# MIT-SPARK/Khronos

Measured on AMD Instinct MI355X. Metric: active-window frames/sec (+ Mvoxel-updates/sec) at 1280x720 RGB-D+labels, 2 cm voxels, higher is better.
Workload: dtype f32

## Files before the change

### khronos_amd/csrc/khr_kernels_fuse.h

```cpp
#pragma once
#include "khr_device.h"

namespace khr {

__device__ inline void interpPixels(float u, float v, int W, int H, int* px, float* du, float* dv) {
  const int u0 = static_cast<int>(floorf(u)), v0 = static_cast<int>(floorf(v));
  const int u1 = min(u0 + 1, W - 1), v1 = min(v0 + 1, H - 1);
  *du = u - static_cast<float>(u0);
  *dv = v - static_cast<float>(v0);
  px[0] = v0 * W + u0;
  px[1] = v1 * W + u0;
  px[2] = v0 * W + u1;
  px[3] = v1 * W + u1;
}

__device__ inline int interpWeights(float du, float dv, bool use_nearest, float* w4) {
  int best;
  if (use_nearest) {
    const int nearest = (du >= 0.5f ? 2 : 0) + (dv >= 0.5f ? 1 : 0);
#pragma unroll
    for (int k = 0; k < 4; ++k) w4[k] = (k == nearest) ? 1.f : 0.f;
    best = nearest;
  } else {
    w4[0] = (1.f - du) * (1.f - dv);
// ... 369 lines not shown
  __syncthreads();
  char* const sink_b = reinterpret_cast<char*>(a.sink) + (static_cast<size_t>(blockIdx.x) * WPW + static_cast<size_t>(wave)) * 256u;
  const bool trk = a.with_tracking != 0;
  const uint32_t first = (blockIdx.x & 7u) * (gridDim.x >> 3) + (blockIdx.x >> 3);
  auto pull = [&]() -> uint32_t {
    uint32_t j = 0u;
    if (lane == 0) j = atomicAdd(&s_q, 1u);
    j = static_cast<uint32_t>(__builtin_amdgcn_readfirstlane(static_cast<int>(j)));
    return first + gridDim.x * j;
  };
  auto descOf = [&](uint32_t i) -> uint4 {
    typedef const FuseList __attribute__((address_space(4))) * FuseListK;
    const char __attribute__((address_space(4)))* kb = (const char __attribute__((address_space(4)))*)__builtin_amdgcn_kernarg_segment_ptr();
    asm volatile("" : "+s"(kb));
    const FuseListK kl = (FuseListK)(kb + ((sizeof(FuseArgs) + 7u) & ~static_cast<size_t>(7)));
    const uint32_t __attribute__((address_space(4)))* const kc = (const uint32_t __attribute__((address_space(4)))*)kl->counts;
    const uint32_t c0 = kc[0], c1 = c0 + kc[1], c2 = c1 + kc[2];
    const DescK la = (DescK)kl->a, lb = (DescK)kl->b;
    const uint32_t cap = kl->cap;
    u4v d;
    if (i < c0) d = la[i];
    else if (i < c1) d = la[cap - 1u - (i - c0)];
    else if (i < c2) d = lb[i - c1];
    else d = lb[cap - 1u - (i - c2)];
    return make_uint4(d.x, d.y, d.z, d.w);
  };

  auto phase1 = [&](FuseItem<VPS, ZR>& it, const uint4 desc) {
    const uint32_t dx = static_cast<uint32_t>(__builtin_amdgcn_readfirstlane(static_cast<int>(desc.x)));
    it.slot = dx & 0xffffffu;
    it.sbi = static_cast<int>(dx >> 24);
    const int bx = __builtin_amdgcn_readfirstlane(static_cast<int>(desc.y));
    const int by = __builtin_amdgcn_readfirstlane(static_cast<int>(desc.z));
    const int bz = __builtin_amdgcn_readfirstlane(static_cast<int>(desc.w));
    const int patch = it.sbi % PATCHES;
    it.z0 = (it.sbi / PATCHES) * ZR;
    const float ox = static_cast<float>(bx) * a.bs, oy = static_cast<float>(by) * a.bs;
    it.oz = static_cast<float>(bz) * a.bs;
    it.lin_xy = patch * 64 + lane;
    const int ix = it.lin_xy % VPS, iy = it.lin_xy / VPS;
    const float px = ox + (static_cast<float>(ix) + 0.5f) * a.vs;
    const float py = oy + (static_cast<float>(iy) + 0.5f) * a.vs;
    float pxy[3];
#pragma unroll
    for (int c = 0; c < 3; ++c) pxy[c] = a.R[3 * c] * px + a.R[3 * c + 1] * py;
    it.pxy2 = pxy[2];
    const char* const dist_b = reinterpret_cast<const char*>(a.dist + it.slot * NV);
    const char* const wgt_b = reinterpret_cast<const char*>(a.weight + it.slot * NV);
#pragma unroll
    for (int k = 0; k < ZR; ++k) {
      const int iz = it.z0 + k;
      const uint32_t lin = static_cast<uint32_t>(it.lin_xy + iz * SL);
      const float pz = it.oz + (static_cast<float>(iz) + 0.5f) * a.vs;
      float pc[3];
#pragma unroll
      for (int c = 0; c < 3; ++c) pc[c] = (pxy[c] + a.R[3 * c + 2] * pz) + a.t[c];
      bool ok = pc[2] > 0.f;
      const float voxel_range = range_mode == 0 ? pc[2] : sqrtf((pc[0] * pc[0] + pc[1] * pc[1]) + pc[2] * pc[2]);
      ok = ok && !(voxel_range < a.min_range || voxel_range > a.max_range);
      const float yz = rcpRefined(pc[2]);
      const float u = divExact(pc[0] * a.fx, pc[2], yz) + a.cx;
      const float v = divExact(pc[1] * a.fy, pc[2], yz) + a.cy;
      ok = ok && (fminf(fminf(u, v), fminf(Wm1 - u, Hm1 - v)) >= 0.f);
      const float uc = ok ? u : 0.f, vc = ok ? v : 0.f;
      const uint32_t u0 = static_cast<uint32_t>(static_cast<int>(uc)), v0 = static_cast<uint32_t>(static_cast<int>(vc));
      const uint32_t v1 = min(v0 + 1u, static_cast<uint32_t>(a.H - 1));
      const uint32_t o0 = __umul24(v0, W4) + u0 * 4u, o1 = __umul24(v1, W4) + u0 * 4u;
      it.ra[k] = *reinterpret_cast<const f2u*>(range_b + o0);
      it.rb[k] = *reinterpret_cast<const f2u*>(range_b + o1);
      it.d[k] = *reinterpret_cast<const float*>(dist_b + lin * 4u);
      it.w[k] = *reinterpret_cast<const float*>(wgt_b + lin * 4u);
      it.u[k] = uc;
      it.v[k] = vc;
      it.z[k] = ok ? voxel_range : -1.f;
      it.yz[k] = yz;
    }
  };

  auto phase2 = [&](FuseItem<VPS, ZR>& cur) {
    const size_t slot = cur.slot;
    char* const dist_b = reinterpret_cast<char*>(a.dist + slot * NV);
    char* const wgt_b = reinterpret_cast<char*>(a.weight + slot * NV);
    char* const lobs_b = reinterpret_cast<char*>(a.last_obs + slot * NV);
    uint32_t cnt = 0;
    bool touched = false;
    bool wrote_neg = false;
    const size_t w0 = slot * static_cast<size_t>(NV / 64) + static_cast<size_t>(cur.z0 * PATCHES + cur.sbi % PATCHES);
    u4v ow_next = trk ? ((DescK)(a.obs + w0))[0] : u4v{0u, 0u, 0u, 0u};
#pragma unroll
    for (int k = 0; k < ZR; ++k) {
      const u4v ow_k = ow_next;
      if (k + 1 < ZR && trk) ow_next = ((DescK)(a.obs + w0))[(k + 1) * PATCHES];
      bool ok = cur.z[k] >= 0.f;
      const int iz = cur.z0 + k;
      const uint32_t lin = static_cast<uint32_t>(cur.lin_xy + iz * SL);
      const float d_old = cur.d[k], w_old = cur.w[k];
      float d_out = d_old, w_out = w_old;
      if (__builtin_amdgcn_ballot_w64(ok) != 0ull) {
      const float uc = cur.u[k], vc = cur.v[k], voxel_range = cur.z[k], yz = cur.yz[k];
      float depth = voxel_range;
      if (range_mode != 0) {
        const float pz = cur.oz + (static_cast<float>(iz) + 0.5f) * a.vs;
        depth = (cur.pxy2 + a.R[8] * pz) + a.t[2];
      }
      const uint32_t u0 = static_cast<uint32_t>(static_cast<int>(uc)), v0 = static_cast<uint32_t>(static_cast<int>(vc));
      const uint32_t v1 = min(v0 + 1u, static_cast<uint32_t>(a.H - 1));
      const float du = __builtin_amdgcn_fractf(uc), dv = __builtin_amdgcn_fractf(vc);
      const uint32_t o0 = v0 * W4 + u0 * 4u, o1 = v1 * W4 + u0 * 4u;
      const bool last_col = u0 >= static_cast<uint32_t>(a.W - 1);
      const float r0 = cur.ra[k].x, r1 = cur.rb[k].x, r2 = last_col ? cur.ra[k].x : cur.ra[k].y, r3 = last_col ? cur.rb[k].x : cur.rb[k].y;
      bool use_nearest = interp == 0;
      if (interp == 2) {
        const float mn = fminf(fminf(r0, r1), fminf(r2, r3));
        const float mx = fmaxf(fmaxf(r0, r1), fmaxf(r2, r3));
        use_nearest = use_nearest || (mx - mn > a.adaptive_diff);
      }
      const bool hi_u = du >= 0.5f, hi_v = dv >= 0.5f;
      const float r_near = hi_u ? (hi_v ? r3 : r2) : (hi_v ? r1 : r0);
      const float omu = 1.f - du, omv = 1.f - dv;
      const float w0 = omu * omv, w1 = omu * dv, w2 = du * omv, w3 = du * dv;
      const float r_bil = ((w0 * r0 + w1 * r1) + w2 * r2) + w3 * r3;
      const float dist_surface = use_nearest ? r_near : r_bil;
      ok = ok && (dist_surface >= a.min_range) && !(dist_surface > a.max_range);
      const float sdf = dist_surface - voxel_range;
      ok = ok && !(sdf < -a.trunc);
      bool in_band = ok && (fabsf(sdf) < a.trunc);
      if (__builtin_expect(a.use_mask && __builtin_amdgcn_ballot_w64(in_band) != 0ull, 0)) {
        int best;
        if (use_nearest) {
          best = (hi_u ? 2 : 0) + (hi_v ? 1 : 0);
        } else {
          best = 0;
          float bw = w0;
          if (w1 > bw) { bw = w1; best = 1; }
          if (w2 > bw) { bw = w2; best = 2; }
          if (w3 > bw) { bw = w3; best = 3; }
        }
        const uint32_t uo = ((best & 2) && !last_col) ? 4u : 0u;
        const uint32_t bo = ((best & 1) ? o1 : o0) + uo;
        if (in_band && *reinterpret_cast<const int32_t*>(reinterpret_cast<const char*>(a.dyn) + bo) != 0) {
          ok = false;
          in_band = false;
        }
      }
      if (__builtin_amdgcn_ballot_w64(ok) != 0ull) {
      float w;
      if (EXACT) {
        const float qd = divExact(a.vs, depth, yz);
        w = fxfy * (qd * qd);
        if (!const_weight) {
          const float z2 = depth * depth;
          w = divExact(w, z2, rcpRefined(z2));
        }
        if (use_dropoff && sdf < -a.dropoff_eps) w = fmaxf(w * divExact(a.trunc + sdf, den, yden), 0.f);
      } else {
        const float qd = a.vs * yz;
        w = fxfy * (qd * qd);
        if (!const_weight) w = w * (yz * yz);
        if (use_dropoff && sdf < -a.dropoff_eps) w = fmaxf(w * ((a.trunc + sdf) * yden), 0.f);
      }
      ok = ok && (w > 0.f);
      in_band = in_band && ok;
      const float sdf_c = fmaxf(fminf(a.trunc, sdf), -a.trunc);
      const float tot = w_old + w;
      float d_new;
      if (EXACT) {
        d_new = divExact(d_old * w_old + sdf_c * w, tot, rcpRefined(tot));
      } else {
        d_new = __builtin_fmaf(d_old, w_old, sdf_c * w) * __builtin_amdgcn_rcpf(tot);
      }
      const float w_new = fminf(tot, a.max_weight);
      if (ok) {
        d_out = d_new;
        w_out = w_new;
      }
      const unsigned long long m_band = __builtin_amdgcn_ballot_w64(in_band);
      wrote_neg = wrote_neg || (__builtin_amdgcn_ballot_w64(ok && d_new < 0.f) != 0ull);
      if (m_band) {
        n_band += static_cast<uint32_t>(__popcll(m_band));
        if (in_band) {
          const uint32_t pos = cnt + __builtin_amdgcn_mbcnt_hi(static_cast<uint32_t>(m_band >> 32),
                                                              __builtin_amdgcn_mbcnt_lo(static_cast<uint32_t>(m_band), 0u));
          uint32_t* const rec = &s_rec[wave][0][pos];
          rec[0] = lin | (use_nearest ? 0x10000u : 0u);
          rec[kRecCap] = __float_as_uint(w);
          rec[2 * kRecCap] = __float_as_uint(a.blend_pre ? w_old : w_new);
          rec[3 * kRecCap] = __float_as_uint(uc);
          rec[4 * kRecCap] = __float_as_uint(vc);
        }
        cnt += static_cast<uint32_t>(__popcll(m_band));
      }
      } else {
        ok = false;
      }
      }
      const unsigned long long m_ok = __builtin_amdgcn_ballot_w64(ok);
      n_upd += static_cast<uint32_t>(__popcll(m_ok));
      touched = touched || (m_ok != 0ull);
      {
        char* const d_b = m_ok != 0ull ? dist_b : sink_b;
        char* const w_b = m_ok != 0ull ? wgt_b : sink_b;
        const uint32_t vo = (m_ok != 0ull ? lin : static_cast<uint32_t>(lane)) * 4u;
        *reinterpret_cast<float*>(d_b + vo) = d_out;
        *reinterpret_cast<float*>(w_b + vo) = w_out;
      }
      {
        const uint64_t bits0 = static_cast<uint64_t>(ow_k.x) | (static_cast<uint64_t>(ow_k.y) << 32);
        const uint64_t stamp0 = static_cast<uint64_t>(ow_k.z) | (static_cast<uint64_t>(ow_k.w) << 32);
        const bool same = stamp0 == a.stamp;
        const uint64_t mat = (m_ok != 0ull && !same) ? (bits0 & ~m_ok) : 0ull;
        const uint64_t nb = m_ok == 0ull ? bits0 : (same ? (bits0 | m_ok) : m_ok);
        const uint64_t ns = m_ok == 0ull ? stamp0 : a.stamp;
        const bool real = trk && mat != 0ull;
        char* const st_b = real ? lobs_b : sink_b;
        const uint32_t first_lin = lin - static_cast<uint32_t>(lane) + static_cast<uint32_t>(__builtin_ctzll(mat | (1ull << 63)));
        const bool mine = ((mat >> static_cast<uint32_t>(lane)) & 1ull) != 0ull;
        const uint32_t so = real ? (mine ? lin : first_lin) * 8u : 0u;
        *reinterpret_cast<uint64_t*>(st_b + so) = stamp0;
        ulonglong2* const wp = trk ? (a.obs + w0 + k * PATCHES) : reinterpret_cast<ulonglong2*>(sink_b + 16);
        *wp = make_ulonglong2(nb, ns);
      }
    }
    const uint32_t item_band = cnt;
    if (__builtin_expect(cnt > 0u, 0)) {
      __builtin_amdgcn_fence(__ATOMIC_RELEASE, "wavefront");
      __builtin_amdgcn_wave_barrier();
      FuseArgsK ka = (FuseArgsK)__builtin_amdgcn_kernarg_segment_ptr();
      asm volatile("" : "+s"(ka));
      const FuseFrameK kf = (FuseFrameK)ka;
      if (ka->band_mode != 0 && fuseBandRowsOk(ka->KS, ka->sem_mode, ka->do_sem, ka->has_color)) {
        fuseBandRows<VPS>(ka, kf, slot, &s_rec[wave][0][0], cnt, lane);
      } else {
        for (uint32_t r = static_cast<uint32_t>(lane); r < cnt; r += 64u) {
          const uint32_t* const rec = &s_rec[wave][0][r];
          fuseBandRecord<VPS>(ka, kf, slot, rec[0], __uint_as_float(rec[kRecCap]), __uint_as_float(rec[2 * kRecCap]),
                              __uint_as_float(rec[3 * kRecCap]), __uint_as_float(rec[4 * kRecCap]));
        }
      }
      __builtin_amdgcn_fence(__ATOMIC_ACQUIRE, "wavefront");
      __builtin_amdgcn_wave_barrier();
      __builtin_amdgcn_s_waitcnt(0x0f70);
    }
    {
      const uint32_t recw = min(item_band, static_cast<uint32_t>(kItemBandMask)) | (touched ? kItemTouched : 0u) | (wrote_neg ? kItemNeg : 0u);
      a.blk_band[slot * kBandSlots + (cur.sbi & (kBandSlots - 1))] = static_cast<uint16_t>(recw);
    }
  };

  uint32_t item = pull();
  if (item < n_items) {
    FuseItem<VPS, ZR> sa, sb;
    uint4 d_cur = descOf(item);
    phase1(sa, d_cur);
    uint32_t item_next = pull();
    uint4 d_next = item_next < n_items ? descOf(item_next) : d_cur;
    while (true) {
      {
        phase1(sb, d_next);
        const uint32_t item_nn = item_next < n_items ? pull() : 0xffffffffu;
        const uint4 d_nn = item_nn < n_items ? descOf(item_nn) : d_next;
        phase2(sa);
        if (item_next >= n_items) break;
        item_next = item_nn;
        d_next = d_nn;
      }
      {
        phase1(sa, d_next);
        const uint32_t item_nn = item_next < n_items ? pull() : 0xffffffffu;
        const uint4 d_nn = item_nn < n_items ? descOf(item_nn) : d_next;
        phase2(sb);
        if (item_next >= n_items) break;
        item_next = item_nn;
        d_next = d_nn;
      }
    }
  }
  if (lane == 0) {
    s_stat[wave][0] = n_upd;
    s_stat[wave][1] = n_band;
  }
  __syncthreads();
  if (threadIdx.x == 0) {
    uint32_t su = 0u, sb2 = 0u;
#pragma unroll
    for (int w = 0; w < WPW; ++w) {
      su += s_stat[w][0];
      sb2 += s_stat[w][1];
    }
    if (su | sb2) {
      a.wg_stats[2 * blockIdx.x] += su;
      a.wg_stats[2 * blockIdx.x + 1] += sb2;
    }
  }
}

__global__ __launch_bounds__(256) void k_fuse_fold(uint32_t* __restrict__ blk_flags, uint16_t* __restrict__ blk_band,
                                                  const uint32_t* __restrict__ max_slot, const uint32_t* gate) {
  if (gate != nullptr && *gate != 0u) return;
  const uint32_t s = blockIdx.x * blockDim.x + threadIdx.x;
  if (s >= *max_slot) return;
  foldItemRecords(blk_flags, blk_band, s);
}

template <int VPS, int ZSPLIT, bool DEFCFG, bool EXACT, int WPW, int MINW>
__global__ __launch_bounds__(64 * WPW, MINW) void k_fuse2(FuseArgs a, FuseList list) {
  constexpr int NV = VPS * VPS * VPS;
  constexpr int SL = VPS * VPS;
  constexpr int PATCHES = SL / 64;
  constexpr int ZR = VPS / ZSPLIT;
  constexpr int CAP = 64 * ZR;
  static_assert(SL % 64 == 0 && VPS % ZSPLIT == 0 && (ZR == 2 || ZR == 4), "bad block shape");
  __shared__ uint32_t s_rec[WPW][5][CAP];
  __shared__ uint32_t s_stat[WPW][2];
  __shared__ uint32_t s_q;
  const int wave = __builtin_amdgcn_readfirstlane(static_cast<int>(threadIdx.x >> 6));
  const int lane = static_cast<int>(threadIdx.x & 63);
  const int range_mode = DEFCFG ? 0 : a.range_mode;
  const int interp = DEFCFG ? 2 : a.interp;
  const bool use_dropoff = DEFCFG ? true : (a.use_dropoff != 0);
  const bool const_weight = DEFCFG ? false : (a.const_weight != 0);
  const float den = a.trunc - a.dropoff_eps;
  const float yden = rcpRefined(den);
  const uint32_t nc0 = list.counts[0], nc1 = nc0 + list.counts[1], nc2 = nc1 + list.counts[2], n_items = nc2 + list.counts[3];
  uint32_t n_upd = 0, n_band = 0;
  if (a.gate != nullptr && *a.gate != 0u) return;
  if (threadIdx.x == 0) s_q = 0u;
  __syncthreads();
  const uint32_t first = (blockIdx.x & 7u) * (gridDim.x >> 3) + (blockIdx.x >> 3);
  auto pull = [&]() -> uint32_t {
    uint32_t j = 0u;
    if (lane == 0) j = atomicAdd(&s_q, 1u);
    j = static_cast<uint32_t>(__builtin_amdgcn_readfirstlane(static_cast<int>(j)));
    return first + gridDim.x * j;
  };
  const DescK la = (DescK)list.a, lb = (DescK)list.b;
  auto descOf = [&](uint32_t i) -> uint4 {
    u4v d;
    if (i < nc0) d = la[i];
    else if (i < nc1) d = la[list.cap - 1u - (i - nc0)];
    else if (i < nc2) d = lb[i - nc1];
    else d = lb[list.cap - 1u - (i - nc2)];
    return make_uint4(d.x, d.y, d.z, d.w);
  };
  uint32_t item = pull();
  uint4 desc = make_uint4(0u, 0u, 0u, 0u);
  if (item < n_items) desc = descOf(item);
  while (item < n_items) {
    const uint32_t item_next = pull();
    uint4 d_next = make_uint4(0u, 0u, 0u, 0u);
    if (item_next < n_items) d_next = descOf(item_next);
    const size_t slot = desc.x & 0xffffffu;
    const int sbi = static_cast<int>(desc.x >> 24);
    const int bx = static_cast<int>(desc.y), by = static_cast<int>(desc.z), bz = static_cast<int>(desc.w);
    const int patch = sbi % PATCHES;
    const int z0 = (sbi / PATCHES) * ZR;
    const float ox = static_cast<float>(bx) * a.bs, oy = static_cast<float>(by) * a.bs, oz = static_cast<float>(bz) * a.bs;
    const int lin_xy = patch * 64 + lane;
    const int ix = lin_xy % VPS, iy = lin_xy / VPS;
    const float px = ox + (static_cast<float>(ix) + 0.5f) * a.vs;
    const float py = oy + (static_cast<float>(iy) + 0.5f) * a.vs;
    char* const dist_b = reinterpret_cast<char*>(a.dist + slot * NV);
    char* const wgt_b = reinterpret_cast<char*>(a.weight + slot * NV);
    char* const lobs_b = reinterpret_cast<char*>(a.last_obs + slot * NV);
    bool touched = false, wrote_neg = false;
    uint32_t cnt = 0;
    const int n_frames = a.n_frames;
    float dreg[ZR], wreg[ZR];
    int lidx[ZR];
#pragma unroll
    for (int k = 0; k < ZR; ++k) {
      const uint32_t lin = static_cast<uint32_t>(lin_xy + (z0 + k) * SL);
      dreg[k] = *reinterpret_cast<const float*>(dist_b + lin * 4u);
      wreg[k] = *reinterpret_cast<const float*>(wgt_b + lin * 4u);
      lidx[k] = -1;
    }
    uint32_t frame_mask = ~0u;
    if (a.item_mask != nullptr) {
      const size_t mi = slot * static_cast<size_t>(PATCHES * ZSPLIT) + static_cast<size_t>(sbi);
      const uint32_t word = *(const uint32_t __attribute__((address_space(4)))*)(a.item_mask + (mi & ~static_cast<size_t>(3)));
      frame_mask = (word >> (8u * static_cast<uint32_t>(mi & 3))) & 0xffu;
      asm volatile("" : "+s"(frame_mask) : : "memory");
      if (lane == 0) a.item_mask[mi] = 0;
    }
    uint32_t fbits = ~0u;
    for (int fi = 0; fi < n_frames; ++fi) {
    if (((frame_mask >> fi) & 1u) == 0u) continue;
    if (a.frame_bits != nullptr) {
      const int gf = fi + a.frame_bit0;
      if ((gf & 31) == 0 || fi == 0) {
        const size_t wi = (slot * static_cast<size_t>(PATCHES * ZSPLIT) + static_cast<size_t>(sbi)) * static_cast<size_t>(a.frame_words) + static_cast<size_t>(gf >> 5);
        fbits = *(const uint32_t __attribute__((address_space(4)))*)(a.frame_bits + wi);
      }
      if (((fbits >> (gf & 31)) & 1u) == 0u) {
        cnt = 0;
        continue;
      }
    }
    FuseFrame F;
    {
      const uint32_t __attribute__((address_space(4)))* const w = (const uint32_t __attribute__((address_space(4)))*)(a.frames + fi);
      uint32_t* const d = reinterpret_cast<uint32_t*>(&F);
#pragma unroll
      for (int i = 0; i < static_cast<int>(sizeof(FuseFrame) / 4); ++i) d[i] = w[i];
    }
    const float Wm1 = static_cast<float>(F.W - 1), Hm1 = static_cast<float>(F.H - 1);
    const float fxfy = F.fx * F.fy;
    const char* const range_b = reinterpret_cast<const char*>(F.range);
    const uint32_t W4 = static_cast<uint32_t>(F.W) * 4u;
    float pxy[3];
#pragma unroll
    for (int c = 0; c < 3; ++c) pxy[c] = F.R[3 * c] * px + F.R[3 * c + 1] * py;
    float uu[ZR], vv[ZR], zz[ZR], yzz[ZR], dd[ZR], ww[ZR];
    f2u ra[ZR], rb[ZR];
    bool okk[ZR];
#pragma unroll
    for (int k = 0; k < ZR; ++k) {
      const int iz = z0 + k;
      const float pz = oz + (static_cast<float>(iz) + 0.5f) * a.vs;
      float pc[3];
#pragma unroll
      for (int c = 0; c < 3; ++c) pc[c] = (pxy[c] + F.R[3 * c + 2] * pz) + F.t[c];
      bool ok = pc[2] > 0.f;
      const float voxel_range = range_mode == 0 ? pc[2] : sqrtf((pc[0] * pc[0] + pc[1] * pc[1]) + pc[2] * pc[2]);
      ok = ok && !(voxel_range < F.min_range || voxel_range > F.max_range);
      const float yz = rcpRefined(pc[2]);
      const float u = divExact(pc[0] * F.fx, pc[2], yz) + F.cx;
      const float v = divExact(pc[1] * F.fy, pc[2], yz) + F.cy;
      ok = ok && (fminf(fminf(u, v), fminf(Wm1 - u, Hm1 - v)) >= 0.f);
      const float uc = ok ? u : 0.f, vc = ok ? v : 0.f;
      const uint32_t u0 = static_cast<uint32_t>(static_cast<int>(uc)), v0 = static_cast<uint32_t>(static_cast<int>(vc));
      const uint32_t v1 = min(v0 + 1u, static_cast<uint32_t>(F.H - 1));
      const uint32_t o0 = v0 * W4 + u0 * 4u, o1 = v1 * W4 + u0 * 4u;
      ra[k] = *reinterpret_cast<const f2u*>(range_b + o0);
      rb[k] = *reinterpret_cast<const f2u*>(range_b + o1);
      dd[k] = dreg[k];
      ww[k] = wreg[k];
      uu[k] = uc;
      vv[k] = vc;
      zz[k] = voxel_range;
      yzz[k] = yz;
      okk[k] = ok;
    }
    cnt = 0;
#pragma unroll
    for (int k = 0; k < ZR; ++k) {
      bool ok = okk[k];
      if (__builtin_amdgcn_ballot_w64(ok) == 0ull) continue;
      const int iz = z0 + k;
      const uint32_t lin = static_cast<uint32_t>(lin_xy + iz * SL);
      const float uc = uu[k], vc = vv[k], voxel_range = zz[k], yz = yzz[k];
      float depth = voxel_range;
      if (range_mode != 0) {
        const float pz = oz + (static_cast<float>(iz) + 0.5f) * a.vs;
        depth = (pxy[2] + F.R[8] * pz) + F.t[2];
      }
      const uint32_t u0 = static_cast<uint32_t>(static_cast<int>(uc)), v0 = static_cast<uint32_t>(static_cast<int>(vc));
      const uint32_t v1 = min(v0 + 1u, static_cast<uint32_t>(F.H - 1));
      const float du = __builtin_amdgcn_fractf(uc), dv = __builtin_amdgcn_fractf(vc);
      const uint32_t o0 = v0 * W4 + u0 * 4u, o1 = v1 * W4 + u0 * 4u;
      const float d_old = dd[k], w_old = ww[k];
      const bool last_col = u0 >= static_cast<uint32_t>(F.W - 1);
      const float r0 = ra[k].x, r1 = rb[k].x, r2 = last_col ? ra[k].x : ra[k].y, r3 = last_col ? rb[k].x : rb[k].y;
      bool use_nearest = interp == 0;
      if (interp == 2) {
        const float mn = fminf(fminf(r0, r1), fminf(r2, r3));
        const float mx = fmaxf(fmaxf(r0, r1), fmaxf(r2, r3));
        use_nearest = use_nearest || (mx - mn > a.adaptive_diff);
      }
      const bool hi_u = du >= 0.5f, hi_v = dv >= 0.5f;
      const float r_near = hi_u ? (hi_v ? r3 : r2) : (hi_v ? r1 : r0);
      const float omu = 1.f - du, omv = 1.f - dv;
      const float w0 = omu * omv, w1 = omu * dv, w2 = du * omv, w3 = du * dv;
      const float r_bil = ((w0 * r0 + w1 * r1) + w2 * r2) + w3 * r3;
      const float dist_surface = use_nearest ? r_near : r_bil;
      ok = ok && (dist_surface >= F.min_range) && !(dist_surface > F.max_range);
      const float sdf = dist_surface - voxel_range;
      ok = ok && !(sdf < -a.trunc);
      bool in_band = ok && (fabsf(sdf) < a.trunc);
      if (__builtin_expect(F.use_mask && __builtin_amdgcn_ballot_w64(in_band) != 0ull, 0)) {
        int best;
        if (use_nearest) {
          best = (hi_u ? 2 : 0) + (hi_v ? 1 : 0);
        } else {
          best = 0;
          float bw = w0;
          if (w1 > bw) { bw = w1; best = 1; }
          if (w2 > bw) { bw = w2; best = 2; }
          if (w3 > bw) { bw = w3; best = 3; }
        }
        const uint32_t uo = ((best & 2) && !last_col) ? 4u : 0u;
        const uint32_t bo = ((best & 1) ? o1 : o0) + uo;
        if (in_band && *reinterpret_cast<const int32_t*>(reinterpret_cast<const char*>(F.dyn) + bo) != 0) {
          ok = false;
          in_band = false;
        }
      }
      if (__builtin_amdgcn_ballot_w64(ok) == 0ull) continue;
      float w;
      if (EXACT) {
        const float qd = divExact(a.vs, depth, yz);
        w = fxfy * (qd * qd);
        if (!const_weight) {
          const float z2 = depth * depth;
          w = divExact(w, z2, rcpRefined(z2));
        }
        if (use_dropoff && sdf < -a.dropoff_eps) w = fmaxf(w * divExact(a.trunc + sdf, den, yden), 0.f);
      } else {
        const float qd = a.vs * yz;
        w = fxfy * (qd * qd);
        if (!const_weight) w = w * (yz * yz);
        if (use_dropoff && sdf < -a.dropoff_eps) w = fmaxf(w * ((a.trunc + sdf) * yden), 0.f);
      }
      ok = ok && (w > 0.f);
      in_band = in_band && ok;
      const float sdf_c = fmaxf(fminf(a.trunc, sdf), -a.trunc);
      const float tot = w_old + w;
      float d_new;
      if (EXACT) {
        d_new = divExact(d_old * w_old + sdf_c * w, tot, rcpRefined(tot));
      } else {
        d_new = __builtin_fmaf(d_old, w_old, sdf_c * w) * __builtin_amdgcn_rcpf(tot);
      }
      const float w_new = fminf(tot, a.max_weight);
      if (ok) {
        dreg[k] = d_new;
        wreg[k] = w_new;
        lidx[k] = fi;
      }
      const unsigned long long m_ok = __builtin_amdgcn_ballot_w64(ok), m_band = __builtin_amdgcn_ballot_w64(in_band);
      n_upd += static_cast<uint32_t>(__popcll(m_ok));
      touched = touched || (m_ok != 0ull);
      wrote_neg = wrote_neg || (__builtin_amdgcn_ballot_w64(ok && d_new < 0.f) != 0ull);
      if (m_band) {
        n_band += static_cast<uint32_t>(__popcll(m_band));
        if (in_band) {
          const uint32_t pos = cnt + __builtin_amdgcn_mbcnt_hi(static_cast<uint32_t>(m_band >> 32),
                                                              __builtin_amdgcn_mbcnt_lo(static_cast<uint32_t>(m_band), 0u));
          uint32_t* const rec = &s_rec[wave][0][pos];
          rec[0] = lin | (use_nearest ? 0x10000u : 0u);
          rec[CAP] = __float_as_uint(w);
          rec[2 * CAP] = __float_as_uint(a.blend_pre ? w_old : w_new);
          rec[3 * CAP] = __float_as_uint(uc);
          rec[4 * CAP] = __float_as_uint(vc);
        }
        cnt += static_cast<uint32_t>(__popcll(m_band));
      }
    }
    if (__builtin_expect(cnt > 0u, 0)) {
      __builtin_amdgcn_fence(__ATOMIC_RELEASE, "wavefront");
      __builtin_amdgcn_wave_barrier();
      FuseArgsK ka = (FuseArgsK)__builtin_amdgcn_kernarg_segment_ptr();
      asm volatile("" : "+s"(ka));
      const FuseFrameK kf = (FuseFrameK)(a.frames + fi);
      if (ka->band_mode != 0 && fuseBandRowsOk(ka->KS, ka->sem_mode, kf->do_sem, kf->has_color)) {
        fuseBandRows<VPS, CAP>(ka, kf, slot, &s_rec[wave][0][0], cnt, lane);
      } else {
        for (uint32_t r = static_cast<uint32_t>(lane); r < cnt; r += 64u) {
          const uint32_t* const rec = &s_rec[wave][0][r];
          fuseBandRecord<VPS>(ka, kf, slot, rec[0], __uint_as_float(rec[CAP]), __uint_as_float(rec[2 * CAP]),
                              __uint_as_float(rec[3 * CAP]), __uint_as_float(rec[4 * CAP]));
        }
      }
      __builtin_amdgcn_fence(__ATOMIC_ACQUIRE, "wavefront");
      __builtin_amdgcn_wave_barrier();
    }
    }
#pragma unroll
    for (int k = 0; k < ZR; ++k) {
      const uint32_t lin = static_cast<uint32_t>(lin_xy + (z0 + k) * SL);
      const unsigned long long m_upd = __builtin_amdgcn_ballot_w64(lidx[k] >= 0);
      if (a.with_tracking && m_upd != 0ull && lane == 0)
        atomicAnd(reinterpret_cast<unsigned long long*>(a.obs + slot * static_cast<size_t>(NV / 64) + (lin >> 6)), ~m_upd);
      if (lidx[k] < 0) continue;
      *reinterpret_cast<float*>(dist_b + lin * 4u) = dreg[k];
      *reinterpret_cast<float*>(wgt_b + lin * 4u) = wreg[k];
      if (a.with_tracking) *reinterpret_cast<uint64_t*>(lobs_b + lin * 8u) = a.frames[lidx[k]].stamp;
    }
    if (lane == 0) {
      if (touched) atomicOr(&a.blk_flags[slot], BLK_UPDATED | BLK_MESH_UPDATED | BLK_TRACKING_UPDATED | (wrote_neg ? BLK_HAS_NEG : 0u));
      a.blk_band[slot * kBandSlots + (sbi & (kBandSlots - 1))] = static_cast<uint16_t>(min(cnt, 65535u));
    }
    item = item_next;
    desc = d_next;
  }
  if (lane == 0) {
    s_stat[wave][0] = n_upd;
    s_stat[wave][1] = n_band;
  }
  __syncthreads();
  if (threadIdx.x == 0) {
    uint32_t su = 0u, sb = 0u;
#pragma unroll
    for (int w = 0; w < WPW; ++w) {
      su += s_stat[w][0];
      sb += s_stat[w][1];
    }
    if (su | sb) {
      a.wg_stats[2 * blockIdx.x] += su;
      a.wg_stats[2 * blockIdx.x + 1] += sb;
    }
  }
}

template <int VPS>
__global__ __launch_bounds__(256) void k_multi_cull(const uint32_t* __restrict__ blk_flags, const int4* __restrict__ blk_index, const uint32_t* __restrict__ n_slots_ptr,
                                                   float vs, float bs, float trunc, const FuseFrame* __restrict__ frames, int n_frames,
                                                   int n_words, uint32_t wpb, uint32_t live_flag, uint32_t* __restrict__ bits) {
  constexpr int kTileSide = 16;
  const uint32_t per_item = static_cast<uint32_t>(n_words) * 32u;
  const uint64_t total = static_cast<uint64_t>(*n_slots_ptr) * wpb * per_item;
  const uint64_t stride = static_cast<uint64_t>(gridDim.x) * blockDim.x;
  for (uint64_t t0 = static_cast<uint64_t>(blockIdx.x) * blockDim.x; t0 < total; t0 += stride) {
    const uint64_t t = t0 + threadIdx.x;
    bool keep = false;
    if (t < total) {
      const uint32_t it = static_cast<uint32_t>(t / per_item);
      const int fr = static_cast<int>(t % per_item);
      const uint32_t slot = it / wpb, item = it % wpb;
      if (fr < n_frames && (blk_flags[slot] & live_flag)) {
        keep = true;
        const FuseFrame& F = frames[fr];
        const int4 bi = blk_index[slot];
        const float margin = 1e-3f;
        const int patches = (VPS * VPS) >> 6, rows = 64 / VPS, zr = VPS / (static_cast<int>(wpb) / patches);
        const int y0 = (static_cast<int>(item) % patches) * rows, z0 = (static_cast<int>(item) / patches) * zr;
        const float lo[3] = {static_cast<float>(bi.x) * bs + 0.5f * vs, static_cast<float>(bi.y) * bs + (static_cast<float>(y0) + 0.5f) * vs,
                             static_cast<float>(bi.z) * bs + (static_cast<float>(z0) + 0.5f) * vs};
        const float ex[3] = {bs - vs, static_cast<float>(rows - 1) * vs, static_cast<float>(zr - 1) * vs};
        float zmin = 1e30f, zmax = -1e30f, umin = 1e30f, umax = -1e30f, vmin = 1e30f, vmax = -1e30f;
        float pcs[8][3];
#pragma unroll
        for (int k = 0; k < 8; ++k) {
          const float x = lo[0] + ((k & 1) ? ex[0] : 0.f), y = lo[1] + ((k & 2) ? ex[1] : 0.f), z = lo[2] + ((k & 4) ? ex[2] : 0.f);
#pragma unroll
          for (int c = 0; c < 3; ++c) pcs[k][c] = ((F.R[3 * c] * x + F.R[3 * c + 1] * y) + F.R[3 * c + 2] * z) + F.t[c];
          zmin = fminf(zmin, pcs[k][2]);
          zmax = fmaxf(zmax, pcs[k][2]);
        }
        if (zmax <= -margin) keep = false;
        if (zmin > F.max_range + margin) keep = false;
        if (zmax < F.min_range - margin) keep = false;
        if (keep && zmin > 0.05f && F.tile_max != nullptr) {
#pragma unroll
          for (int k = 0; k < 8; ++k) {
            const float iz = __builtin_amdgcn_rcpf(pcs[k][2]);
            const float u = (pcs[k][0] * F.fx) * iz + F.cx, v = (pcs[k][1] * F.fy) * iz + F.cy;
            umin = fminf(umin, u); umax = fmaxf(umax, u);
            vmin = fminf(vmin, v); vmax = fmaxf(vmax, v);
          }
          if (umax < -2.f || vmax < -2.f || umin > static_cast<float>(F.W) + 1.f || vmin > static_cast<float>(F.H) + 1.f) {
            keep = false;
          } else {
            const int tx0 = max(0, (static_cast<int>(floorf(umin)) - 2) / kTileSide);
            const int ty0 = max(0, (static_cast<int>(floorf(vmin)) - 2) / kTileSide);
            const int tx1 = min(F.tw - 1, (static_cast<int>(ceilf(umax)) + 3) / kTileSide);
            const int ty1 = min(F.th - 1, (static_cast<int>(ceilf(vmax)) + 3) / kTileSide);
            const int nx = tx1 - tx0 + 1, ny = ty1 - ty0 + 1;
            if (nx > 0 && ny > 0 && nx * ny <= 96) {
              float mr = 0.f;
              for (int ty = ty0; ty <= ty1; ++ty)
                for (int tx = tx0; tx <= tx1; ++tx) mr = fmaxf(mr, F.tile_max[ty * F.tw + tx]);
              if (mr < zmin - trunc - margin) keep = false;
            }
          }
        }
      }
    }
    const unsigned long long b = __ballot(keep);
    const uint32_t lane = threadIdx.x & 63u;
    if (t < total && (lane & 31u) == 0u) bits[t >> 5] = static_cast<uint32_t>(lane ? (b >> 32) : b);
  }
}

__global__ __launch_bounds__(1024) void k_multi_order(const uint32_t* __restrict__ blk_flags, const int4* __restrict__ blk_index, const uint32_t* __restrict__ n_slots_ptr,
                                                     const uint32_t* __restrict__ bits, int n_words, int n_frames, uint32_t wpb, uint32_t live_flag,
                                                     FuseList out) {
  __shared__ uint32_t s_cnt[4], s_off[4];
  const uint32_t n_items = *n_slots_ptr * wpb;
  if (threadIdx.x < 4) s_cnt[threadIdx.x] = 0u;
  __syncthreads();
  const uint32_t it = blockIdx.x * blockDim.x + threadIdx.x;
  uint32_t n = 0u, cls = 0u, pos = 0u;
  if (it < n_items && (blk_flags[it / wpb] & live_flag))
    for (int w = 0; w < n_words; ++w) n += static_cast<uint32_t>(__popc(bits[static_cast<size_t>(it) * n_words + w]));
  if (n) {
    const uint32_t q = 4u * n, f = static_cast<uint32_t>(n_frames);
    cls = q >= 3u * f ? 0u : (q >= 2u * f ? 1u : (q >= f ? 2u : 3u));
    pos = atomicAdd(&s_cnt[cls], 1u);
  }
  __syncthreads();
  if (threadIdx.x < 4) s_off[threadIdx.x] = s_cnt[threadIdx.x] ? atomicAdd(&out.counts[threadIdx.x], s_cnt[threadIdx.x]) : 0u;
  __syncthreads();
  if (n) {
    const uint32_t slot = it / wpb;
    const int4 bi = blk_index[slot];
    *fuseDescPtr(out, cls, s_off[cls] + pos) =
        make_uint4(slot | ((it % wpb) << 24), static_cast<uint32_t>(bi.x), static_cast<uint32_t>(bi.y), static_cast<uint32_t>(bi.z));
  }
}

struct FuseFrameSet {
  FuseFrame f[kMaxTick];
};
__global__ __launch_bounds__(256) void k_copy_words(const uint32_t* __restrict__ src, uint32_t* __restrict__ dst, uint32_t n) {
  const uint32_t i = blockIdx.x * blockDim.x + threadIdx.x;
  if (i < n) dst[i] = src[i];
}
__global__ void k_put_frames(FuseFrameSet s, FuseFrame* __restrict__ dst, int n) {
  const uint32_t* const src = reinterpret_cast<const uint32_t*>(&s);
  uint32_t* const d = reinterpret_cast<uint32_t*>(dst);
  for (uint32_t i = threadIdx.x; i < static_cast<uint32_t>(n) * (sizeof(FuseFrame) / 4); i += blockDim.x) d[i] = src[i];
}

}
```

Baseline: 3964.

## Prefetch depth-image samples for upcoming frames into an LDS ring in fuse kernel

For 8-voxel blocks, the per-frame fusion loop now issues global_load_lds requests for the range-image pixel pairs of the next one or two allowed frames into a per-wave LDS ring. It waits on vmcnt only for the frame about to be folded, so gather latency overlaps with the fold math of earlier frames. The cost is extra LDS per block, which may lower occupancy, plus hand-written waitcnt and ds_read assembly that is fragile. Separately, k_multi_order becomes a grid-stride loop so it can run with fewer blocks.

```diff
diff --git a/khronos_amd/csrc/khr_kernels_fuse.h b/khronos_amd/csrc/khr_kernels_fuse.h
--- a/khronos_amd/csrc/khr_kernels_fuse.h
+++ b/khronos_amd/csrc/khr_kernels_fuse.h
@@ -695,6 +695,11 @@
   foldItemRecords(blk_flags, blk_band, s);
 }
 
+constexpr int kMultiRing = 3;
+template <int N>
+__device__ __forceinline__ void waitVm() {
+  asm volatile("s_waitcnt vmcnt(%0)" : : "n"(N) : "memory");
+}
 template <int VPS, int ZSPLIT, bool DEFCFG, bool EXACT, int WPW, int MINW>
 __global__ __launch_bounds__(64 * WPW, MINW) void k_fuse2(FuseArgs a, FuseList list) {
   constexpr int NV = VPS * VPS * VPS;
@@ -702,8 +707,10 @@
   constexpr int PATCHES = SL / 64;
   constexpr int ZR = VPS / ZSPLIT;
   constexpr int CAP = 64 * ZR;
+  constexpr int RING = VPS == 8 ? kMultiRing : 0;
   static_assert(SL % 64 == 0 && VPS % ZSPLIT == 0 && (ZR == 2 || ZR == 4), "bad block shape");
   __shared__ uint32_t s_rec[WPW][5][CAP];
+  __shared__ uint32_t s_ring[RING > 0 ? WPW : 1][RING > 0 ? RING : 1][4 * ZR][64];
   __shared__ uint32_t s_stat[WPW][2];
   __shared__ uint32_t s_q;
   const int wave = __builtin_amdgcn_readfirstlane(static_cast<int>(threadIdx.x >> 6));
@@ -776,64 +783,60 @@
       if (lane == 0) a.item_mask[mi] = 0;
     }
     uint32_t fbits = ~0u;
-    for (int fi = 0; fi < n_frames; ++fi) {
-    if (((frame_mask >> fi) & 1u) == 0u) continue;
-    if (a.frame_bits != nullptr) {
-      const int gf = fi + a.frame_bit0;
-      if ((gf & 31) == 0 || fi == 0) {
-        const size_t wi = (slot * static_cast<size_t>(PATCHES * ZSPLIT) + static_cast<size_t>(sbi)) * static_cast<size_t>(a.frame_words) + static_cast<size_t>(gf >> 5);
-        fbits = *(const uint32_t __attribute__((address_space(4)))*)(a.frame_bits + wi);
-      }
-      if (((fbits >> (gf & 31)) & 1u) == 0u) {
-        cnt = 0;
-        continue;
-      }
-    }
-    FuseFrame F;
-    {
+    int zeroed = -1, folded = -1;
+    auto allowed = [&](int fi) -> bool {
+      if (((frame_mask >> fi) & 1u) == 0u) return false;
+      if (a.frame_bits != nullptr) {
+        const int gf = fi + a.frame_bit0;
+        if ((gf & 31) == 0 || fi == 0) {
+          const size_t wi = (slot * static_cast<size_t>(PATCHES * ZSPLIT) + static_cast<size_t>(sbi)) * static_cast<size_t>(a.frame_words) + static_cast<size_t>(gf >> 5);
+          fbits = *(const uint32_t __attribute__((address_space(4)))*)(a.frame_bits + wi);
+        }
+        if (((fbits >> (gf & 31)) & 1u) == 0u) {
+          zeroed = fi;
+          return false;
+        }
+      }
+      return true;
+    };
+    auto frameOf = [&](int fi) -> FuseFrame {
+      FuseFrame F;
       const uint32_t __attribute__((address_space(4)))* const w = (const uint32_t __attribute__((address_space(4)))*)(a.frames + fi);
       uint32_t* const d = reinterpret_cast<uint32_t*>(&F);
 #pragma unroll
       for (int i = 0; i < static_cast<int>(sizeof(FuseFrame) / 4); ++i) d[i] = w[i];
-    }
-    const float Wm1 = static_cast<float>(F.W - 1), Hm1 = static_cast<float>(F.H - 1);
-    const float fxfy = F.fx * F.fy;
-    const char* const range_b = reinterpret_cast<const char*>(F.range);
-    const uint32_t W4 = static_cast<uint32_t>(F.W) * 4u;
-    float pxy[3];
-#pragma unroll
-    for (int c = 0; c < 3; ++c) pxy[c] = F.R[3 * c] * px + F.R[3 * c + 1] * py;
-    float uu[ZR], vv[ZR], zz[ZR], yzz[ZR], dd[ZR], ww[ZR];
-    f2u ra[ZR], rb[ZR];
-    bool okk[ZR];
-#pragma unroll
-    for (int k = 0; k < ZR; ++k) {
+      return F;
+    };
+    auto project = [&](const FuseFrame& F, const float (&pxy)[3], int k, float& uc, float& vc, float& voxel_range, float& yz) -> bool {
+      const float Wm1 = static_cast<float>(F.W - 1), Hm1 = static_cast<float>(F.H - 1);
       const int iz = z0 + k;
       const float pz = oz + (static_cast<float>(iz) + 0.5f) * a.vs;
       float pc[3];
 #pragma unroll
       for (int c = 0; c < 3; ++c) pc[c] = (pxy[c] + F.R[3 * c + 2] * pz) + F.t[c];
       bool ok = pc[2] > 0.f;
-      const float voxel_range = range_mode == 0 ? pc[2] : sqrtf((pc[0] * pc[0] + pc[1] * pc[1]) + pc[2] * pc[2]);
+      voxel_range = range_mode == 0 ? pc[2] : sqrtf((pc[0] * pc[0] + pc[1] * pc[1]) + pc[2] * pc[2]);
       ok = ok && !(voxel_range < F.min_range || voxel_range > F.max_range);
-      const float yz = rcpRefined(pc[2]);
+      yz = rcpRefined(pc[2]);
       const float u = divExact(pc[0] * F.fx, pc[2], yz) + F.cx;
       const float v = divExact(pc[1] * F.fy, pc[2], yz) + F.cy;
       ok = ok && (fminf(fminf(u, v), fminf(Wm1 - u, Hm1 - v)) >= 0.f);
-      const float uc = ok ? u : 0.f, vc = ok ? v : 0.f;
+      uc = ok ? u : 0.f;
+      vc = ok ? v : 0.f;
+      return ok;
+    };
+    auto pairOffsets = [&](const FuseFrame& F, float uc, float vc, uint32_t& o0, uint32_t& o1) {
+      const uint32_t W4 = static_cast<uint32_t>(F.W) * 4u;
       const uint32_t u0 = static_cast<uint32_t>(static_cast<int>(uc)), v0 = static_cast<uint32_t>(static_cast<int>(vc));
       const uint32_t v1 = min(v0 + 1u, static_cast<uint32_t>(F.H - 1));
-      const uint32_t o0 = v0 * W4 + u0 * 4u, o1 = v1 * W4 + u0 * 4u;
-      ra[k] = *reinterpret_cast<const f2u*>(range_b + o0);
-      rb[k] = *reinterpret_cast<const f2u*>(range_b + o1);
-      dd[k] = dreg[k];
-      ww[k] = wreg[k];
-      uu[k] = uc;
-      vv[k] = vc;
-      zz[k] = voxel_range;
-      yzz[k] = yz;
-      okk[k] = ok;
-    }
+      o0 = v0 * W4 + u0 * 4u;
+      o1 = v1 * W4 + u0 * 4u;
+    };
+    auto fold = [&](int fi, const FuseFrame& F, const float (&pxy)[3], const float (&uu)[ZR], const float (&vv)[ZR], const float (&zz)[ZR],
+                    const float (&yzz)[ZR], const bool (&okk)[ZR], const f2u (&ra)[ZR], const f2u (&rb)[ZR]) {
+    const float fxfy = F.fx * F.fy;
+    const uint32_t W4 = static_cast<uint32_t>(F.W) * 4u;
+    folded = fi;
     cnt = 0;
 #pragma unroll
     for (int k = 0; k < ZR; ++k) {
@@ -851,7 +854,7 @@
       const uint32_t v1 = min(v0 + 1u, static_cast<uint32_t>(F.H - 1));
       const float du = __builtin_amdgcn_fractf(uc), dv = __builtin_amdgcn_fractf(vc);
       const uint32_t o0 = v0 * W4 + u0 * 4u, o1 = v1 * W4 + u0 * 4u;
-      const float d_old = dd[k], w_old = ww[k];
+      const float d_old = dreg[k], w_old = wreg[k];
       const bool last_col = u0 >= static_cast<uint32_t>(F.W - 1);
       const float r0 = ra[k].x, r1 = rb[k].x, r2 = last_col ? ra[k].x : ra[k].y, r3 = last_col ? rb[k].x : rb[k].y;
       bool use_nearest = interp == 0;
@@ -957,7 +960,118 @@
       __builtin_amdgcn_fence(__ATOMIC_ACQUIRE, "wavefront");
       __builtin_amdgcn_wave_barrier();
     }
-    }
+    };
+    if constexpr (RING == 0) {
+      for (int fi = 0; fi < n_frames; ++fi) {
+        if (!allowed(fi)) continue;
+        const FuseFrame F = frameOf(fi);
+        const char* const range_b = reinterpret_cast<const char*>(F.range);
+        float pxy[3];
+#pragma unroll
+        for (int c = 0; c < 3; ++c) pxy[c] = F.R[3 * c] * px + F.R[3 * c + 1] * py;
+        float uu[ZR], vv[ZR], zz[ZR], yzz[ZR];
+        f2u ra[ZR], rb[ZR];
+        bool okk[ZR];
+#pragma unroll
+        for (int k = 0; k < ZR; ++k) {
+          okk[k] = project(F, pxy, k, uu[k], vv[k], zz[k], yzz[k]);
+          uint32_t o0, o1;
+          pairOffsets(F, uu[k], vv[k], o0, o1);
+          ra[k] = *reinterpret_cast<const f2u*>(range_b + o0);
+          rb[k] = *reinterpret_cast<const f2u*>(range_b + o1);
+        }
+        fold(fi, F, pxy, uu, vv, zz, yzz, okk, ra, rb);
+      }
+    } else {
+      static_assert(ZR == 2 && RING >= 2 && RING <= 3, "the ring walk is built for two z steps per lane");
+      typedef __attribute__((address_space(1))) const void* GPtr;
+      typedef __attribute__((address_space(3))) void* LPtr;
+      auto request = [&](int fi, uint32_t s) {
+        const FuseFrame F = frameOf(fi);
+        const char* const range_b = reinterpret_cast<const char*>(F.range);
+        float pxy[3];
+#pragma unroll
+        for (int c = 0; c < 3; ++c) pxy[c] = F.R[3 * c] * px + F.R[3 * c + 1] * py;
+#pragma unroll
+        for (int k = 0; k < ZR; ++k) {
+          float uc, vc, vr, yz;
+          project(F, pxy, k, uc, vc, vr, yz);
+          uint32_t o0, o1;
+          pairOffsets(F, uc, vc, o0, o1);
+          uint32_t* const dst = &s_ring[wave][s][4 * k][0];
+          __builtin_amdgcn_global_load_lds((GPtr)(range_b + o0), (LPtr)(dst), 4, 0, 0);
+          __builtin_amdgcn_global_load_lds((GPtr)(range_b + o0 + 4u), (LPtr)(dst + 64), 4, 0, 0);
+          __builtin_amdgcn_global_load_lds((GPtr)(range_b + o1), (LPtr)(dst + 128), 4, 0, 0);
+          __builtin_amdgcn_global_load_lds((GPtr)(range_b + o1 + 4u), (LPtr)(dst + 192), 4, 0, 0);
+        }
+      };
+      int scan = 0;
+      auto nextAllowed = [&]() -> int {
+        while (scan < n_frames) {
+          const int fi = scan++;
+          if (allowed(fi)) return fi;
+        }
+        return -1;
+      };
+      int fq[RING];
+#pragma unroll
+      for (int j = 0; j + 1 < RING; ++j) fq[j] = -1;
+      fq[RING - 1] = nextAllowed();
+      if (fq[RING - 1] >= 0) request(fq[RING - 1], 0u);
+#pragma unroll
+      for (int k = 0; k < ZR; ++k) asm volatile("" : "+v"(dreg[k]), "+v"(wreg[k]));
+      uint32_t sw = 1u, sl = 0u;
+      int fill = RING - 2;
+      for (;;) {
+#pragma unroll
+        for (int j = 0; j + 1 < RING; ++j) fq[j] = fq[j + 1];
+        fq[RING - 1] = nextAllowed();
+        if (fq[RING - 1] >= 0) request(fq[RING - 1], sw);
+        sw = sw + 1u == static_cast<uint32_t>(RING) ? 0u : sw + 1u;
+        if (fill > 0) {
+          --fill;
+          continue;
+        }
+        if (fq[0] < 0) break;
+        const int fi = fq[0];
+        const FuseFrame F = frameOf(fi);
+        float pxy[3];
+#pragma unroll
+        for (int c = 0; c < 3; ++c) pxy[c] = F.R[3 * c] * px + F.R[3 * c + 1] * py;
+        float uu[ZR], vv[ZR], zz[ZR], yzz[ZR];
+        f2u ra[ZR], rb[ZR];
+        bool okk[ZR];
+#pragma unroll
+        for (int k = 0; k < ZR; ++k) okk[k] = project(F, pxy, k, uu[k], vv[k], zz[k], yzz[k]);
+        int ahead = 0;
+#pragma unroll
+        for (int j = 1; j < RING; ++j) ahead += fq[j] >= 0 ? 1 : 0;
+        if (ahead == 0) waitVm<0>();
+        else if (ahead == 1) waitVm<4 * ZR>();
+        else waitVm<8 * ZR>();
+        {
+          const uint32_t at = static_cast<uint32_t>(reinterpret_cast<uintptr_t>((LPtr)(&s_ring[wave][sl][0][lane])));
+          float r[8];
+          asm volatile(
+              "ds_read_b32 %0, %8\n\tds_read_b32 %1, %8 offset:256\n\tds_read_b32 %2, %8 offset:512\n\tds_read_b32 %3, %8 offset:768\n\t"
+              "ds_read_b32 %4, %8 offset:1024\n\tds_read_b32 %5, %8 offset:1280\n\tds_read_b32 %6, %8 offset:1536\n\t"
+              "ds_read_b32 %7, %8 offset:1792\n\ts_waitcnt lgkmcnt(0)"
+              : "=&v"(r[0]), "=&v"(r[1]), "=&v"(r[2]), "=&v"(r[3]), "=&v"(r[4]), "=&v"(r[5]), "=&v"(r[6]), "=&v"(r[7])
+              : "v"(at)
+              : "memory");
+#pragma unroll
+          for (int k = 0; k < ZR; ++k) {
+            ra[k].x = r[4 * k];
+            ra[k].y = r[4 * k + 1];
+            rb[k].x = r[4 * k + 2];
+            rb[k].y = r[4 * k + 3];
+          }
+        }
+        fold(fi, F, pxy, uu, vv, zz, yzz, okk, ra, rb);
+        sl = sl + 1u == static_cast<uint32_t>(RING) ? 0u : sl + 1u;
+      }
+    }
+    if (zeroed > folded) cnt = 0;
 #pragma unroll
     for (int k = 0; k < ZR; ++k) {
       const uint32_t lin = static_cast<uint32_t>(lin_xy + (z0 + k) * SL);
@@ -1070,25 +1184,28 @@
                                                      FuseList out) {
   __shared__ uint32_t s_cnt[4], s_off[4];
   const uint32_t n_items = *n_slots_ptr * wpb;
-  if (threadIdx.x < 4) s_cnt[threadIdx.x] = 0u;
-  __syncthreads();
-  const uint32_t it = blockIdx.x * blockDim.x + threadIdx.x;
-  uint32_t n = 0u, cls = 0u, pos = 0u;
-  if (it < n_items && (blk_flags[it / wpb] & live_flag))
-    for (int w = 0; w < n_words; ++w) n += static_cast<uint32_t>(__popc(bits[static_cast<size_t>(it) * n_words + w]));
-  if (n) {
-    const uint32_t q = 4u * n, f = static_cast<uint32_t>(n_frames);
-    cls = q >= 3u * f ? 0u : (q >= 2u * f ? 1u : (q >= f ? 2u : 3u));
-    pos = atomicAdd(&s_cnt[cls], 1u);
-  }
-  __syncthreads();
-  if (threadIdx.x < 4) s_off[threadIdx.x] = s_cnt[threadIdx.x] ? atomicAdd(&out.counts[threadIdx.x], s_cnt[threadIdx.x]) : 0u;
-  __syncthreads();
-  if (n) {
-    const uint32_t slot = it / wpb;
-    const int4 bi = blk_index[slot];
-    *fuseDescPtr(out, cls, s_off[cls] + pos) =
-        make_uint4(slot | ((it % wpb) << 24), static_cast<uint32_t>(bi.x), static_cast<uint32_t>(bi.y), static_cast<uint32_t>(bi.z));
+  for (uint32_t base = blockIdx.x * blockDim.x; base < n_items; base += gridDim.x * blockDim.x) {
+    if (threadIdx.x < 4) s_cnt[threadIdx.x] = 0u;
+    __syncthreads();
+    const uint32_t it = base + threadIdx.x;
+    uint32_t n = 0u, cls = 0u, pos = 0u;
+    if (it < n_items && (blk_flags[it / wpb] & live_flag))
+      for (int w = 0; w < n_words; ++w) n += static_cast<uint32_t>(__popc(bits[static_cast<size_t>(it) * n_words + w]));
+    if (n) {
+      const uint32_t q = 4u * n, f = static_cast<uint32_t>(n_frames);
+      cls = q >= 3u * f ? 0u : (q >= 2u * f ? 1u : (q >= f ? 2u : 3u));
+      pos = atomicAdd(&s_cnt[cls], 1u);
+    }
+    __syncthreads();
+    if (threadIdx.x < 4) s_off[threadIdx.x] = s_cnt[threadIdx.x] ? atomicAdd(&out.counts[threadIdx.x], s_cnt[threadIdx.x]) : 0u;
+    __syncthreads();
+    if (n) {
+      const uint32_t slot = it / wpb;
+      const int4 bi = blk_index[slot];
+      *fuseDescPtr(out, cls, s_off[cls] + pos) =
+          make_uint4(slot | ((it % wpb) << 24), static_cast<uint32_t>(bi.x), static_cast<uint32_t>(bi.y), static_cast<uint32_t>(bi.z));
+    }
+    __syncthreads();
   }
 }
 
```

Result: slower. 3746 (-5.5%).
